# mcogoni/supersdr

Hardware: AMD Instinct MI355X
Metric: real-time IQ channels sustained (WF+demod) (higher is better)
Workload: dtype f32

## Files before the change

### supersdr_amd/csrc/ssdr_audio_dev.h

```cpp
#pragma once
#include "ssdr_math.h"
#include "ssdr_kernels.h"

constexpr int OCT = 10;
constexpr int NOCT = (SSDR_HIST + SSDR_FRAME) / 8;
constexpr int HOCT = SSDR_HIST / 8;
typedef uint32_t u32x4 __attribute__((ext_vector_type(4)));

SSDR_DEV void lds_sync()
{
    __builtin_amdgcn_fence(__ATOMIC_RELEASE, "wavefront");
    __builtin_amdgcn_wave_barrier();
    __builtin_amdgcn_fence(__ATOMIC_ACQUIRE, "wavefront");
}

template <int CTRL, int ROWMASK>
SSDR_DEV float dpp(float identity, float x)
{
    return __int_as_float(__builtin_amdgcn_update_dpp(__float_as_int(identity), __float_as_int(x), CTRL, ROWMASK, 0xF, false));
}
SSDR_DEV float vmax(float a, float b)
{
    float r;
    asm("v_max_f32 %0, %1, %2" : "=v"(r) : "v"(a), "v"(b));
    return r;
}
SSDR_DEV float vmax3(float a, float b, float c)
{
    float r;
    asm("v_max3_f32 %0, %1, %2, %3" : "=v"(r) : "v"(a), "v"(b), "v"(c));
    return r;
}
SSDR_DEV float vmax3_abs(float a, float b, float c)
{
    float r;
    asm("v_max3_f32 %0, %1, |%2|, |%3|" : "=v"(r) : "v"(a), "v"(b), "v"(c));
    return r;
}
SSDR_DEV uint32_t lane63_u(uint32_t x) { return (uint32_t)__builtin_amdgcn_readlane((int)x, 63); }
SSDR_DEV uint32_t from_prev_lane_u(uint32_t lane0_value, uint32_t x)
{
    return (uint32_t)__builtin_amdgcn_update_dpp((int)lane0_value, (int)x, 0x138, 0xF, 0xF, false);
}
typedef short s16x2 __attribute__((ext_vector_type(2)));
typedef unsigned short u16x2 __attribute__((ext_vector_type(2)));
SSDR_DEV uint32_t iq_power(uint32_t raw)
{
    uint32_t p;
    asm("v_dot2_i32_i16 %0, %1, %1, 0" : "=v"(p) : "v"(raw));
    return p;
}
SSDR_DEV float lane63(float x) { return __int_as_float(__builtin_amdgcn_readlane(__float_as_int(x), 63)); }
SSDR_DEV float from_prev_lane(float lane0_value, float x) { return dpp<0x138, 0xF>(lane0_value, x); }

#define SSDR_SCAN6(STEP) STEP("row_shr:1", "0xf") STEP("row_shr:2", "0xf") STEP("row_shr:4", "0xf") STEP("row_shr:8", "0xf") \
                         STEP("row_bcast:15", "0xa") STEP("row_bcast:31", "0xc")
#define SSDR_DPP(C, M) " " C " row_mask:" M " bank_mask:0xf"

SSDR_DEV float scan_max(float x)
{
#define STEP(C, M) asm("s_nop 1\n\tv_max_f32_dpp %0, %0, %0" SSDR_DPP(C, M) : "+v"(x));
    SSDR_SCAN6(STEP)
#undef STEP
    return x;
}
SSDR_DEV float scan_sum(float x)
{
#define STEP(C, M) asm("s_nop 1\n\tv_add_f32_dpp %0, %0, %0" SSDR_DPP(C, M) : "+v"(x));
    SSDR_SCAN6(STEP)
#undef STEP
    return x;
}
SSDR_DEV void scan_affine(float &A, float &B)
{
#define STEP(C, M) asm("s_nop 1\n\tv_fmac_f32_dpp %1, %1, %0" SSDR_DPP(C, M) "\n\tv_mul_f32_dpp %0, %0, %0" SSDR_DPP(C, M) : "+v"(A), "+v"(B));
    SSDR_SCAN6(STEP)
#undef STEP
}

struct Nco {
    uint32_t dphi;
    float cs, ss;
    float qc, qs;
    float tc, ts;
};
SSDR_DEV void nco_setup(Nco &n, uint32_t dphi, int l, int block = 8)
{
    n.dphi = dphi;
    ssdr_phasor32(dphi, n.cs, n.ss);
    ssdr_phasor32((uint32_t)(block * l) * dphi, n.qc, n.qs);
    n.tc = 1.0f; n.ts = 0.0f;
}
SSDR_DEV void nco_frame_table(Nco &n, uint32_t phase_of_frame, int l, int frame = SSDR_FRAME)
{
    ssdr_phasor32(phase_of_frame + (uint32_t)(frame * l) * n.dphi, n.tc, n.ts);
}
SSDR_DEV float lane_f(float x, uint32_t lane) { return __int_as_float(__builtin_amdgcn_readlane(__float_as_int(x), (int)lane)); }
SSDR_DEV void nco_block(const Nco &n, uint32_t f, float &c, float &s)
{
    const float fc = lane_f(n.tc, f & 63u), fs = lane_f(n.ts, f & 63u);
    c = fmaf(fc, n.qc, -(fs * n.qs));
    s = fmaf(fs, n.qc, fc * n.qs);
}
SSDR_DEV void phasor_mul(float ac, float as, float bc, float bs, float &c, float &s)
{
    c = fmaf(ac, bc, -(as * bs));
    s = fmaf(as, bc, ac * bs);
}

template <bool CLIP, int N = 8>
SSDR_DEV void mix8(const uint32_t (&rw)[N], float c, float s, float cs, float ss, float2 (&z)[N], float &amax)
{
#pragma unroll
    for (int j = 0; j < N; j++) {
        const float xr = (float)(int16_t)(rw[j] & 0xFFFFu);
        const float xi = (float)((int32_t)rw[j] >> 16);
        if (CLIP) amax = vmax3_abs(amax, xr, xi);
        z[j] = make_float2(fmaf(xr, c, xi * s), fmaf(xi, c, -(xr * s)));
        const float cn = fmaf(c, cs, -(s * ss)), sn = fmaf(s, cs, c * ss);
        c = cn; s = sn;
    }
}

template <bool CLIP>
SSDR_DEV void mix8_carry(const uint32_t *rw, float &c, float &s, float cs, float ss, float2 (&z)[8], float &amax)
{
#pragma unroll
    for (int j = 0; j < 8; j++) {
        const float xr = (float)(int16_t)(rw[j] & 0xFFFFu);
        const float xi = (float)((int32_t)rw[j] >> 16);
        if (CLIP) amax = vmax3_abs(amax, xr, xi);
        z[j] = make_float2(fmaf(xr, c, xi * s), fmaf(xi, c, -(xr * s)));
        const float cn = fmaf(c, cs, -(s * ss)), sn = fmaf(s, cs, c * ss);
        c = cn; s = sn;
    }
}

SSDR_DEV void load_oct(const float2 *z, int q, float2 (&v)[8])
{
    const float4 *p = reinterpret_cast<const float4 *>(z + q * OCT);
#pragma unroll
    for (int i = 0; i < 4; i++) {
        const float4 t = p[i];
        v[2 * i] = make_float2(t.x, t.y);
        v[2 * i + 1] = make_float2(t.z, t.w);
    }
}

SSDR_DEV void store_oct(float2 *z, int q, const float2 (&v)[8])
{
    float4 *p = reinterpret_cast<float4 *>(z + q * OCT);
#pragma unroll
    for (int i = 0; i < 4; i++) p[i] = make_float4(v[2 * i].x, v[2 * i].y, v[2 * i + 1].x, v[2 * i + 1].y);
}

template <int K0, int NK>
SSDR_DEV void fir_taps(const float *h, const float2 (&A)[8], const float2 (&B)[8], float (&yr)[8], float (&yi)[8])
{
#pragma unroll
    for (int kk = K0; kk < K0 + NK; kk++) {
#pragma unroll
        for (int j = 0; j < 8; j++) {
            const float2 v = (j - kk >= 0) ? A[(j - kk) & 7] : B[(8 + j - kk) & 7];
            yr[j] = fmaf(h[kk], v.x, yr[j]);
            yi[j] = fmaf(h[kk], v.y, yi[j]);
        }
    }
}


struct AgcK { float c0, c1, knee, d8; uint32_t K; };

template <bool INTEGER_POWER>
SSDR_DEV void demod_am(const float (&p)[8], float &dc, float (&aud)[8])
{
    constexpr float DC_APOW[8] = SSDR_DC_APOW_INIT;
    float env[8], loc[8];
    float s = 0.0f;
#pragma unroll
    for (int j = 0; j < 8; j++) {
        env[j] = INTEGER_POWER ? ssdr_sqrt_rn_int(p[j]) : ssdr_sqrt_rn(p[j]);
        s = fmaf(SSDR_DC_A, s, SSDR_DC_AL * env[j]);
        loc[j] = s;
    }
    float Asc = DC_APOW[7], Bsc = s;
    scan_affine(Asc, Bsc);
    const float Ae = from_prev_lane(1.0f, Asc), Be = from_prev_lane(0.0f, Bsc);
    const float carry = fmaf(Ae, dc, Be);
    float m = 0.0f;
#pragma unroll
    for (int j = 0; j < 8; j++) {
        m = fmaf(DC_APOW[j], carry, loc[j]);
        aud[j] = env[j] - m;
    }
    dc = lane63(m);
}

SSDR_DEV void demod_ssb(const float (&yr)[8], const float (&yi)[8], float c, float s, float cs2, float ss2, float (&aud)[8])
{
#pragma unroll
    for (int j = 0; j < 8; j++) {
        aud[j] = fmaf(yr[j], c, -(yi[j] * s));
        const float cn = fmaf(c, cs2, -(s * ss2)), sn = fmaf(s, cs2, c * ss2);
        c = cn; s = sn;
    }
}

SSDR_DEV void demod_fm(const float (&yr)[8], const float (&yi)[8], float prev_re, float prev_im, float kfm, float (&aud)[8])
{
    float pr = from_prev_lane(prev_re, yr[7]), pi = from_prev_lane(prev_im, yi[7]);
#pragma unroll
    for (int j = 0; j < 8; j++) {
        const float dr = fmaf(yr[j], pr, yi[j] * pi);
        const float di = fmaf(yi[j], pr, -(yr[j] * pi));
        aud[j] = ssdr_atan2p(di, dr) * kfm;
        pr = yr[j]; pi = yi[j];
    }
}

SSDR_DEV float block_peak(const float (&p)[8])
{
    return vmax3(vmax3(vmax3(p[0], p[1], p[2]), p[3], p[4]), vmax3(p[5], p[6], p[7]), SSDR_P_FLOOR);
}

SSDR_DEV float agc_pack_store(const float (&p)[8], const float (&aud)[8], int l, const AgcK &k, float &agc_d,
                              float (&agc_m)[8], int16_t *dst, float pm_known = -1.0f)
{
    const float pm = pm_known >= 0.0f ? pm_known : block_peak(p);
    const float al = ssdr_log2p(pm);
    const float fl = (float)l;
    const float d8 = k.d8;
    float e;
    if (k.K == 0) {
        const float P = scan_max(fmaf(fl, d8, al));
        e = vmax(fmaf(-fl, d8, P), fmaf(-(fl + 1.0f), d8, agc_d));
        agc_d = lane63(e);
    } else {
        const float P = scan_max(al);
        float maxM = agc_m[0], mK = agc_m[0];
#pragma unroll
        for (int i = 1; i < 8; i++)
            if ((uint32_t)i < k.K) { maxM = fmaxf(maxM, agc_m[i]); mK = agc_m[i]; }
        e = vmax(vmax(P, maxM), fmaf(-(fl + 1.0f), d8, agc_d));
        agc_d = fmaxf(fmaf(-64.0f, d8, agc_d), mK);
#pragma unroll
        for (int i = 7; i > 0; i--) agc_m[i] = agc_m[i - 1];
        agc_m[0] = lane63(P);
    }
    const float g = ssdr_exp2p(fmaf(k.c1, vmax(e, k.knee), k.c0));
    u32x4 w;
#pragma unroll
    for (int j = 0; j < 8; j += 2) {
        const int i0 = __float2int_rn(aud[j] * g), i1 = __float2int_rn(aud[j + 1] * g);
        w[j >> 1] = __builtin_bit_cast(uint32_t, __builtin_amdgcn_cvt_pk_i16(i0, i1));
    }
    SSDR_NT_STORE(w, reinterpret_cast<u32x4 *>(dst));
    return g;
}

SSDR_DEV void iq_pack_store(const float (&yr)[8], const float (&yi)[8], float g, uint32_t *dst)
{
    u32x4 w0, w1;
#pragma unroll
    for (int j = 0; j < 8; j++) {
        const uint32_t v = __builtin_bit_cast(uint32_t, __builtin_amdgcn_cvt_pk_i16(__float2int_rn(yr[j] * g), __float2int_rn(yi[j] * g)));
        if (j < 4) w0[j] = v; else w1[j - 4] = v;
    }
    SSDR_NT_STORE(w0, reinterpret_cast<u32x4 *>(dst));
    SSDR_NT_STORE(w1, reinterpret_cast<u32x4 *>(dst) + 1);
}

SSDR_DEV void rssi_flag_step(const float (&p)[8], bool clip, uint32_t f, uint32_t n_frames, int l, float cal,
                             float &rssi_sum, uint32_t &flag_keep, float *rssi_row, uint8_t *flag_row)
{
    float ps = p[0];
#pragma unroll
    for (int j = 1; j < 8; j++) ps = ps + p[j];
    const float tot = lane63(scan_sum(ps));
    if ((f & 63u) == (uint32_t)l) { rssi_sum = tot; flag_keep = clip ? 1u : 0u; }
    if ((f & 63u) == 63u || f + 1 == n_frames) {
        if ((uint32_t)l <= (f & 63u)) {
            rssi_row[(f & ~63u) + l] = fmaf(ssdr_log2p(fmaxf(rssi_sum, 1e-20f)) - 39.0f, SSDR_DB_PER_LOG2, cal);
            flag_row[(f & ~63u) + l] = (uint8_t)flag_keep;
        }
    }
}

SSDR_DEV bool wave_any(bool x) { return __builtin_amdgcn_ballot_w64(x) != 0ull; }

SSDR_DEV bool raw_clipped(const uint32_t (&rw)[8])
{
    bool c = false;
#pragma unroll
    for (int j = 0; j < 8; j++) {
        const int lo = (int16_t)(rw[j] & 0xFFFFu), hi = (int32_t)rw[j] >> 16;
        c = c || lo >= 32767 || lo <= -32767 || hi >= 32767 || hi <= -32767;
    }
    return c;
}

SSDR_DEV uint32_t scan_add_u(uint32_t x)
{
#define STEP(C, M) asm("s_nop 1\n\tv_add_u32_dpp %0, %0, %0" SSDR_DPP(C, M) : "+v"(x));
    SSDR_SCAN6(STEP)
#undef STEP
    return x;
}
SSDR_DEV uint32_t scan_max_u(uint32_t x)
{
#define STEP(C, M) asm("s_nop 1\n\tv_max_u32_dpp %0, %0, %0" SSDR_DPP(C, M) : "+v"(x));
    SSDR_SCAN6(STEP)
#undef STEP
    return x;
}

struct NbRun { uint32_t gate, thresh, s1, s2, left; };

template <int N>
SSDR_DEV uint32_t nb_frame(uint32_t (&rw)[N], int l, NbRun &s, bool &clip)
{
    constexpr uint32_t M = 64u * N;
    constexpr int SHIFT = __builtin_ctz(M);
    const uint32_t lmin = s.s1 < s.s2 ? s.s1 : s.s2;
    const uint64_t t64 = (uint64_t)s.thresh * lmin;
    const uint32_t tc = (t64 == 0 || t64 >= 0xFFFFFFFFull) ? 0xFFFFFFFFu : (uint32_t)t64;
    uint32_t part = 0, trig = 0;
    u16x2 rails = {0xFFFFu, 0xFFFFu};
#pragma unroll
    for (int j = 0; j < N; j++) {
        const uint32_t p = iq_power(rw[j]);
        part += p >> SHIFT;
        trig |= (uint32_t)(p > tc) << j;
        rails = __builtin_elementwise_min(rails, __builtin_bit_cast(u16x2, rw[j]) + (u16x2){32769u, 32769u});
    }
    clip = wave_any(rails.x < 3u || rails.y < 3u);
    const uint32_t n0 = (uint32_t)(N * l);
    const uint32_t le = trig ? n0 + (31u - (uint32_t)__builtin_clz(trig)) + s.gate : 0u;
    const uint32_t sc = scan_max_u(le);
    const uint32_t from_left = from_prev_lane_u(0u, sc);
    const uint32_t e = s.left > from_left ? s.left : from_left;
    int d = (int)e - (int)n0;
    uint32_t mask = 0;
#pragma unroll
    for (int j = 0; j < N; j++) {
        d = (trig >> j) & 1u ? j + (int)s.gate : d;
        const bool b = j < d;
        mask |= (uint32_t)b << j;
        rw[j] = b ? 0u : rw[j];
    }
    const uint32_t sum = lane63_u(scan_add_u(part));
    const uint32_t last = lane63_u(sc);
    const uint32_t ef = s.left > last ? s.left : last;
    s.left = ef > M ? ef - M : 0u;
    s.s2 = s.s1;
    s.s1 = sum;
    return mask;
}
```

### supersdr_amd/csrc/ssdr_wf.hip

```cpp
#include "ssdr_math.h"
#include "ssdr_kernels.h"
#include "ssdr_audio_dev.h"
#include "ssdr_wf_dev.h"

namespace {

constexpr int WAVES = SSDR_WF_BLOCK / 64;
constexpr int LDS_TOTAL = LDS_XCH + WAVES * 2 * XCH_FLOATS * 4;
static_assert(LDS_TOTAL <= 163840, "LDS budget");

template <bool AVG, bool HOP>
__global__ __launch_bounds__(SSDR_WF_BLOCK, SSDR_WF_WAVES_PER_EU) void ssdr_wf_kernel(SsdrWfArgs a)
{
    __shared__ __attribute__((aligned(16))) unsigned char smem[LDS_TOTAL];
    load_tables(smem, a.win, a.tw_stage, a.lut);

    const int lane = threadIdx.x & 63, wave = __builtin_amdgcn_readfirstlane(threadIdx.x >> 6);
    const int h = lane >> 5, l = lane & 31;
    float *xch_wave = reinterpret_cast<float *>(smem + LDS_XCH) + wave * 2 * XCH_FLOATS;
    const unsigned char *lut = smem + LDS_LUT0;
    const uint32_t n_pairs = (a.n_ch + 1) >> 1;
    const uint32_t run = HOP ? a.grp_run : 1u;
    const uint32_t n_runs = (a.n_groups + run - 1) / run;
    const uint32_t n_items = n_pairs * n_runs;
    const uint32_t wave_stride = gridDim.x * WAVES;

    for (uint32_t item = blockIdx.x * WAVES + wave; item < n_items; item += wave_stride) {
      uint32_t pair, g_begin, g_end;
      if (HOP) {
          pair = item / n_runs;
          g_begin = (item - pair * n_runs) * run;
          g_end = min(g_begin + run, a.n_groups);
      } else {
          g_begin = item / n_pairs;
          pair = item - g_begin * n_pairs;
          g_end = g_begin + 1;
      }
      const uint32_t n_trips = HOP ? g_end - g_begin : 1u;
      for (uint32_t trip = 0; trip < n_trips; trip++) {
        const uint32_t grp = g_begin + trip;
        uint32_t pair_now = __builtin_amdgcn_readfirstlane(pair);
        asm volatile("" : "+s"(pair_now));
        const WfItem it = wf_item(a, pair_now, grp, h);
        const float calq = a.consts[it.ch].wf_cal_lin * SSDR_LUT_SCALE;
        uint32_t acc[AVG ? 16 : 1];
#pragma unroll
        for (int j = 0; j < (AVG ? 16 : 1); j++) acc[j] = 0;
        constexpr uint32_t LINE_STEP = HOP ? SSDR_NFFT / 2 : SSDR_NFFT;
        const uint32_t *src = a.iq + (uint64_t)it.ch * a.ch_stride + (uint64_t)it.l0 * LINE_STEP + l;

        for (uint32_t line = it.l0; line < it.l1; line++, src += LINE_STEP) {
            f32x2 z[32];
            uint32_t raw[32];
            if (HOP) load_line_halves(line ? src - SSDR_NFFT / 2 : a.tail + (uint64_t)it.ch * (SSDR_NFFT / 2) + l, src, raw);
            else load_line(src, raw);
            if (SSDR_PRIO_WF) prio_compute_phase();
            window_line(raw, smem, l, z);
            SCHED_FENCE();
            fft_line<AVG>(z, smem, xch_wave, h, l);
            if (SSDR_PRIO_WF) prio_latency_phase();

            if (AVG) {
                quantise32(z, calq, lut, [&](int j, uint32_t q01) { acc[j] += q01; });
            } else {
                uint32_t q[16];
                quantise32(z, calq, lut, [&](int j, uint32_t q01) { q[j] = q01; });
                int16_t *x16 = reinterpret_cast<int16_t *>(xch_wave + opaque(h) * XCH_FLOATS) + opaque(l);
#pragma unroll
                for (int j = 0; j < 16; j++) {
                    x16[32 * (j + 16)] = (int16_t)(q[j] & 0xFFFFu);
                    x16[32 * j] = (int16_t)(q[j] >> 16);
                }
            }
        }

        float *xch = xch_wave + opaque(h) * XCH_FLOATS;
        if (AVG) {
            int16_t *x16 = reinterpret_cast<int16_t *>(xch) + opaque(l);
#pragma unroll
            for (int j = 0; j < 16; j++) {
                x16[32 * (j + 16)] = (int16_t)(acc[j] & 0xFFFFu);
                x16[32 * j] = (int16_t)(acc[j] >> 16);
            }
        }
        wave_lds_sync();
        const u32x4 *x128 = reinterpret_cast<const u32x4 *>(xch);
        int16_t *dst = it.complete ? a.out + ((uint64_t)it.grp * a.n_ch + it.ch) * SSDR_NFFT
                                   : a.acc_out + (uint64_t)it.ch * SSDR_NFFT;
        const int16_t *cin = a.acc_in + (uint64_t)it.ch * SSDR_NFFT;
#pragma unroll
        for (int q = 0; q < 4; q++) {
            u32x4 v = x128[q * 32 + l];
            if (AVG && it.carry_in)
                v += reinterpret_cast<const u32x4 *>(cin)[q * 32 + l];
            if (it.ch_ok) SSDR_NT_STORE(v, reinterpret_cast<u32x4 *>(dst) + q * 32 + l);
        }
        wave_lds_sync();
      }
    }
}

template <bool HOP, bool AVG = false>
__global__ __launch_bounds__(SSDR_WF_BLOCK, SSDR_WF_WAVES_PER_EU) void ssdr_fused_am_kernel(SsdrFusedArgs fa)
{
    __shared__ __attribute__((aligned(16))) unsigned char smem[LDS_TOTAL];
    const SsdrWfArgs &a = fa.wf;
    const SsdrAudioArgs &u = fa.au;
    load_tables(smem, a.win, a.tw_stage, a.lut);

    const int lane = threadIdx.x & 63, wave = __builtin_amdgcn_readfirstlane(threadIdx.x >> 6);
    const int h = lane >> 5, l = lane & 31;
    float *xch_wave = reinterpret_cast<float *>(smem + LDS_XCH) + wave * 2 * XCH_FLOATS;
    uint32_t *qbuf = reinterpret_cast<uint32_t *>(xch_wave);
    const unsigned char *lut = smem + LDS_LUT0;
    const uint32_t n_pairs = (a.n_ch + 1) >> 1;
    const uint32_t wave_stride = gridDim.x * WAVES;
    const uint32_t n_frames = u.n_frames;

    for (uint32_t pair = blockIdx.x * WAVES + wave; pair < n_pairs; pair += wave_stride) {
        const uint32_t ch_raw = 2 * pair + h;
        const bool ch_ok = ch_raw < a.n_ch;
        const uint32_t ch = ch_ok ? ch_raw : a.n_ch - 1;
        const float cal_wf = a.consts[ch].wf_cal_lin * SSDR_LUT_SCALE;
        const uint32_t n_sub = (2 * pair + 1 < a.n_ch) ? 2u : 1u;

        float rssi_sum[2] = {0.0f, 0.0f};
        uint32_t flag_keep[2] = {0u, 0u};
        auto pad = [&](int c, int i) -> float & { return xch_wave[c * XCH_FLOATS + 33 * (i + 16) + 32]; };
        if (lane < 2) {
            const uint32_t cc = min(2 * pair + (uint32_t)lane, a.n_ch - 1);
            const ssdr_chan_state st = u.state[cc];
            pad(lane, 0) = st.dc;
            pad(lane, 1) = st.agc_d;
#pragma unroll
            for (int i = 0; i < 8; i++) pad(lane, 2 + i) = st.agc_m[i];
            const uint4 t = *reinterpret_cast<const uint4 *>(u.hist + (size_t)cc * SSDR_HIST + SSDR_HIST - 4);
            pad(lane, 10) = __uint_as_float(iq_power(t.x)); pad(lane, 11) = __uint_as_float(iq_power(t.y));
            pad(lane, 12) = __uint_as_float(iq_power(t.z)); pad(lane, 13) = __uint_as_float(iq_power(t.w));
        }
        wave_lds_sync();

        const uint32_t *src = a.iq + (uint64_t)ch * a.ch_stride + l;
        uint32_t last_raw31 = 0;
        uint32_t acc[AVG ? 16 : 1];
#pragma unroll
        for (int j = 0; j < (AVG ? 16 : 1); j++) acc[j] = 0;
        constexpr uint32_t LINE_STEP = HOP ? SSDR_NFFT / 2 : SSDR_NFFT;
        constexpr int FRAMES_PER_LINE = HOP ? 1 : 2;
        for (uint32_t line = 0; line < a.n_lines; line++, src += LINE_STEP) {
            float dc[2], agc_d[2], agc_m[2][8];
            uint32_t tail_q[2][4];
#pragma unroll
            for (int c = 0; c < 2; c++) {
                dc[c] = pad(c, 0); agc_d[c] = pad(c, 1);
#pragma unroll
                for (int i = 0; i < 8; i++) agc_m[c][i] = pad(c, 2 + i);
#pragma unroll
                for (int i = 0; i < 4; i++) tail_q[c][i] = __float_as_uint(pad(c, 10 + i));
            }
            wave_lds_sync();
            {
                const uint32_t lw = opaque(lane);
                u32x4 t[2][4];
#pragma unroll
                for (int c = 0; c < 2; c++) {
                    uint32_t pair_now = __builtin_amdgcn_readfirstlane(pair);
                    asm volatile("" : "+s"(pair_now));
                    const uint32_t cc = min(2 * pair_now + (uint32_t)c, a.n_ch - 1);
                    const uint32_t *row = a.iq + (uint64_t)cc * a.ch_stride + (uint64_t)line * LINE_STEP;
                    if (HOP) {
                        const uint32_t *older = line ? row - SSDR_NFFT / 2 : a.tail + (uint64_t)cc * (SSDR_NFFT / 2);
#pragma unroll
                        for (int i = 0; i < 2; i++) t[c][i] = SSDR_NT_LOAD(reinterpret_cast<const u32x4 *>(older) + 64 * i + lw);
#pragma unroll
                        for (int i = 0; i < 2; i++) t[c][2 + i] = reinterpret_cast<const u32x4 *>(row)[64 * i + lw];
                    } else {
#pragma unroll
                        for (int i = 0; i < 4; i++) t[c][i] = SSDR_NT_LOAD(reinterpret_cast<const u32x4 *>(row) + 64 * i + lw);
                    }
                }
                SCHED_FENCE();
#pragma unroll
                for (int c = 0; c < 2; c++)
#pragma unroll
                    for (int i = 0; i < 4; i++) reinterpret_cast<u32x4 *>(qbuf + c * XCH_FLOATS)[64 * i + lw] = t[c][i];
                SCHED_FENCE();
            }
            wave_lds_sync();
            prio_latency_phase();
#pragma unroll
            for (int c = 0; c < 2; c++) {
                if ((uint32_t)c >= n_sub) continue;
                uint32_t pair_now = __builtin_amdgcn_readfirstlane(pair);
                asm volatile("" : "+s"(pair_now));
                const uint32_t cc = 2 * pair_now + c;
                const ssdr_chan_consts &kc = u.consts[cc];
                const AgcK agc_c = {kc.agc_c0, kc.agc_c1, kc.agc_knee, kc.agc_delta8, kc.hang_frames};
                const float cal_c = kc.smeter_cal_db;
#pragma unroll
                for (int f = 0; f < FRAMES_PER_LINE; f++) {
                    const uint32_t frame = HOP ? line : 2 * line + f;
                    const u32x4 *qp = reinterpret_cast<const u32x4 *>(qbuf + c * XCH_FLOATS + SSDR_FRAME * (HOP ? 1 : f)) + 2 * opaque(lane);
                    const u32x4 q0 = qp[0], q1 = qp[1];
                    const uint32_t rw[8] = {q0.x, q0.y, q0.z, q0.w, q1.x, q1.y, q1.z, q1.w};
                    uint32_t qv[8], d[8];
#pragma unroll
                    for (int j = 0; j < 8; j++) qv[j] = iq_power(rw[j]);
                    float p[8], aud[8];
#pragma unroll
                    for (int j = 0; j < 4; j++) { d[j] = from_prev_lane_u(tail_q[c][j], qv[4 + j]); d[4 + j] = qv[j]; }
#pragma unroll
                    for (int j = 0; j < 4; j++) tail_q[c][j] = lane63_u(qv[4 + j]);
#pragma unroll
                    for (int j = 0; j < 8; j++) p[j] = (float)d[j];
                    const float pmx = block_peak(p);
                    const bool trig = wave_any(pmx >= 1073676160.0f) || tail_q[c][0] >= 0x3FFF0001u || tail_q[c][1] >= 0x3FFF0001u ||
                                      tail_q[c][2] >= 0x3FFF0001u || tail_q[c][3] >= 0x3FFF0001u;
                    const bool clip = trig ? wave_any(raw_clipped(rw)) : false;
                    demod_am<true>(p, dc[c], aud);
                    agc_pack_store(p, aud, lane, agc_c, agc_d[c], agc_m[c], u.pcm + ((uint64_t)cc * n_frames + frame) * SSDR_FRAME + 8 * lane, pmx);
                    rssi_flag_step(p, clip, frame, n_frames, lane, cal_c, rssi_sum[c], flag_keep[c],
                                   u.rssi + (uint64_t)cc * n_frames, u.flags + (uint64_t)cc * n_frames);
                }
            }
            wave_lds_sync();
            prio_compute_phase();
            uint32_t raw[32];
            {
                const uint32_t *q = qbuf + opaque(h) * XCH_FLOATS + opaque(l);
#pragma unroll
                for (int r = 0; r < 32; r++) raw[r] = q[32 * r];
            }
            wave_lds_sync();
            if (lane < 2) {
#pragma unroll
                for (int c = 0; c < 2; c++) {
                    if (lane != c) continue;
                    pad(c, 0) = dc[c]; pad(c, 1) = agc_d[c];
#pragma unroll
                    for (int i = 0; i < 8; i++) pad(c, 2 + i) = agc_m[c][i];
#pragma unroll
                    for (int i = 0; i < 4; i++) pad(c, 10 + i) = __uint_as_float(tail_q[c][i]);
                }
            }
            wave_lds_sync();
            SCHED_FENCE();
            if (line + 1 == a.n_lines && ch_ok) {
#pragma unroll
                for (int r = 28; r < 32; r++) u.hist[(size_t)ch * SSDR_HIST + 32 * (r - 28) + l] = raw[r];
            }
            last_raw31 = raw[31];
            uint32_t qn[16];
            f32x2 z[32];
            window_line(raw, smem, l, z);
            SCHED_FENCE();
            fft_line<true>(z, smem, xch_wave, h, l);
            prio_latency_phase();
            if (AVG) quantise32(z, cal_wf, lut, [&](int j, uint32_t q01) { acc[j] += q01; });
            else quantise32(z, cal_wf, lut, [&](int j, uint32_t q01) { qn[j] = q01; });
            const uint32_t pos = a.phase + line;
            const bool group_done = !AVG || (pos + 1) % a.n_avg == 0;
            const bool last_line = line + 1 == a.n_lines;
            if (group_done || last_line) {
                float *xch = xch_wave + opaque(h) * XCH_FLOATS;
                int16_t *x16 = reinterpret_cast<int16_t *>(xch) + opaque(l);
#pragma unroll
                for (int j = 0; j < 16; j++) {
                    const uint32_t v = AVG ? acc[j] : qn[j];
                    x16[32 * (j + 16)] = (int16_t)(v & 0xFFFFu);
                    x16[32 * j] = (int16_t)(v >> 16);
                }
                wave_lds_sync();
                const u32x4 *x128 = reinterpret_cast<const u32x4 *>(xch);
                const uint32_t grp = AVG ? pos / a.n_avg : line;
                int16_t *dst = group_done ? a.out + ((uint64_t)grp * a.n_ch + ch) * SSDR_NFFT : a.acc_out + (uint64_t)ch * SSDR_NFFT;
                const bool carry_in = AVG && grp == 0 && a.phase != 0;
                const int16_t *cin = a.acc_in + (uint64_t)ch * SSDR_NFFT;
#pragma unroll
                for (int q = 0; q < 4; q++) {
                    u32x4 v = x128[q * 32 + l];
                    if (carry_in) v += reinterpret_cast<const u32x4 *>(cin)[q * 32 + l];
                    if (ch_ok) SSDR_NT_STORE(v, reinterpret_cast<u32x4 *>(dst) + q * 32 + l);
                }
                wave_lds_sync();
                if (AVG) {
#pragma unroll
                    for (int j = 0; j < 16; j++) acc[j] = 0;
                }
            }
        }

        if (a.n_lines) {
#pragma unroll
            for (int c = 0; c < 2; c++) {
                if ((uint32_t)c >= n_sub) continue;
                const uint32_t cc = 2 * pair + c;
                const ssdr_chan_consts &kc = u.consts[cc];
                ssdr_chan_state st = u.state[cc];
                const uint32_t phi_last = st.phi1 + (uint32_t)(SSDR_FRAME * (n_frames - 1)) * kc.dphi1;
                float fc, fs, qc, qs, bc, bs, cs, ss;
                ssdr_phasor32(phi_last, fc, fs);
                ssdr_phasor32((uint32_t)(8 * 63) * kc.dphi1, qc, qs);
                ssdr_phasor32(kc.dphi1, cs, ss);
                phasor_mul(fc, fs, qc, qs, bc, bs);
#pragma unroll
                for (int j = 0; j < 3; j++) { const float cn = fmaf(bc, cs, -(bs * ss)), sn = fmaf(bs, cs, bc * ss); bc = cn; bs = sn; }
                const float xr = (float)(int16_t)(last_raw31 & 0xFFFFu), xi = (float)((int32_t)last_raw31 >> 16);
                const float zr = fmaf(xr, bc, xi * bs) + 0.0f, zi = fmaf(xi, bc, -(xr * bs)) + 0.0f;
                st.prev_re = lane_f(zr, 32 * c + 27);
                st.prev_im = lane_f(zi, 32 * c + 27);
                st.phi1 += (uint32_t)(SSDR_FRAME * n_frames) * kc.dphi1;
                st.phi2 += (uint32_t)(SSDR_FRAME * n_frames) * kc.dphi2;
                st.dc = pad(c, 0); st.agc_d = pad(c, 1);
#pragma unroll
                for (int i = 0; i < 8; i++) st.agc_m[i] = pad(c, 2 + i);
                if (lane == 0) u.state[cc] = st;
            }
        }
    }
}

__global__ __launch_bounds__(256) void ssdr_quant_selftest_kernel(const float *thr_g, const uint32_t *lut_g,
                                                                    unsigned long long *mismatch)
{
    __shared__ __attribute__((aligned(16))) unsigned char smem[LDS_LUT_END + 16 + 1024];
    float *s_thr = reinterpret_cast<float *>(smem + ((LDS_LUT_END + 15) & ~15));
    uint32_t *s_lut = reinterpret_cast<uint32_t *>(smem + LDS_LUT0);
    for (int i = threadIdx.x; i < 256; i += blockDim.x) s_thr[i] = thr_g[i];
    for (int i = threadIdx.x; i < SSDR_LUT_N; i += blockDim.x) s_lut[i] = lut_g[i];
    __syncthreads();
    unsigned long long bad = 0;
    const unsigned char *lut = smem + LDS_LUT0;
    const uint64_t stride = (uint64_t)gridDim.x * blockDim.x;
    for (uint64_t u = (uint64_t)blockIdx.x * blockDim.x + threadIdx.x; u < 0x7F800000ull; u += stride) {
        const float p = __uint_as_float((uint32_t)u);
        int lo = 0, hi = 255;
        while (lo < hi) {
            const int mid = (lo + hi + 1) >> 1;
            if (s_thr[mid] <= p) lo = mid; else hi = mid - 1;
        }
        float pc;
        asm("v_mul_f32_e64 %0, %1, %2 clamp" : "=v"(pc) : "v"(p), "v"(SSDR_LUT_SCALE));
        bad += (quantise(pc, lut) != (uint32_t)lo);
    }
    if (bad) atomicAdd(mismatch, bad);
}

}

hipError_t ssdr_launch_wf(const SsdrWfArgs &a, uint32_t grid, hipStream_t stream)
{
    const dim3 g(grid), b(SSDR_WF_BLOCK);
    if (a.tail) {
        if (a.n_avg > 1) hipLaunchKernelGGL((ssdr_wf_kernel<true, true>), g, b, 0, stream, a);
        else hipLaunchKernelGGL((ssdr_wf_kernel<false, true>), g, b, 0, stream, a);
    } else {
        if (a.n_avg > 1) hipLaunchKernelGGL((ssdr_wf_kernel<true, false>), g, b, 0, stream, a);
        else hipLaunchKernelGGL((ssdr_wf_kernel<false, false>), g, b, 0, stream, a);
    }
    return hipGetLastError();
}

hipError_t ssdr_launch_fused_am(const SsdrFusedArgs &a, uint32_t grid, hipStream_t stream)
{
    if (a.wf.n_avg > 1) {
        if (a.wf.tail) hipLaunchKernelGGL((ssdr_fused_am_kernel<true, true>), dim3(grid), dim3(SSDR_WF_BLOCK), 0, stream, a);
        else hipLaunchKernelGGL((ssdr_fused_am_kernel<false, true>), dim3(grid), dim3(SSDR_WF_BLOCK), 0, stream, a);
    } else {
        if (a.wf.tail) hipLaunchKernelGGL((ssdr_fused_am_kernel<true, false>), dim3(grid), dim3(SSDR_WF_BLOCK), 0, stream, a);
        else hipLaunchKernelGGL((ssdr_fused_am_kernel<false, false>), dim3(grid), dim3(SSDR_WF_BLOCK), 0, stream, a);
    }
    return hipGetLastError();
}

hipError_t ssdr_fused_blocks_per_cu(int *blocks)
{
    int b[4] = {0, 0, 0, 0};
    hipError_t e = hipOccupancyMaxActiveBlocksPerMultiprocessor(&b[0], ssdr_fused_am_kernel<false, false>, SSDR_WF_BLOCK, 0);
    if (e == hipSuccess) e = hipOccupancyMaxActiveBlocksPerMultiprocessor(&b[1], ssdr_fused_am_kernel<true, false>, SSDR_WF_BLOCK, 0);
    if (e == hipSuccess) e = hipOccupancyMaxActiveBlocksPerMultiprocessor(&b[2], ssdr_fused_am_kernel<false, true>, SSDR_WF_BLOCK, 0);
    if (e == hipSuccess) e = hipOccupancyMaxActiveBlocksPerMultiprocessor(&b[3], ssdr_fused_am_kernel<true, true>, SSDR_WF_BLOCK, 0);
    *blocks = b[0];
    for (int i = 1; i < 4; i++) *blocks = b[i] < *blocks ? b[i] : *blocks;
    return e;
}

hipError_t ssdr_wf_blocks_per_cu(int *blocks)
{
    int b[4] = {0, 0, 0, 0};
    hipError_t e = hipOccupancyMaxActiveBlocksPerMultiprocessor(&b[0], ssdr_wf_kernel<false, false>, SSDR_WF_BLOCK, 0);
    if (e == hipSuccess) e = hipOccupancyMaxActiveBlocksPerMultiprocessor(&b[1], ssdr_wf_kernel<true, false>, SSDR_WF_BLOCK, 0);
    if (e == hipSuccess) e = hipOccupancyMaxActiveBlocksPerMultiprocessor(&b[2], ssdr_wf_kernel<false, true>, SSDR_WF_BLOCK, 0);
    if (e == hipSuccess) e = hipOccupancyMaxActiveBlocksPerMultiprocessor(&b[3], ssdr_wf_kernel<true, true>, SSDR_WF_BLOCK, 0);
    if (e != hipSuccess) return e;
    *blocks = b[0];
    for (int i = 1; i < 4; i++) *blocks = b[i] < *blocks ? b[i] : *blocks;
    return hipSuccess;
}

hipError_t ssdr_launch_quant_selftest(const float *thr, const uint32_t *lut, unsigned long long *mismatch, hipStream_t stream)
{
    hipLaunchKernelGGL(ssdr_quant_selftest_kernel, dim3(2048), dim3(256), 0, stream, thr, lut, mismatch);
    return hipGetLastError();
}
```

Before: 43.88 million.

## Keep AM demod AGC/DC carry state in scalar registers and a dedicated LDS slot

The per-channel DC, AGC decay and tail-power carries used to be saved to and reloaded from the LDS exchange pad on every line, which cost extra wave barriers. They are now held in wave-uniform scalar registers (readfirstlane plus asm pinning), and the 8-entry AGC hang history moves to its own small LDS region read as float4. This removes a load/sync and a store/sync per line and replaces the runtime-indexed hang loop with a switch over fixed window sizes. The cost is more LDS per workgroup, still checked against a two-workgroup-per-CU budget, and more SGPR pressure.

```diff
diff --git a/supersdr_amd/csrc/ssdr_audio_dev.h b/supersdr_amd/csrc/ssdr_audio_dev.h
--- a/supersdr_amd/csrc/ssdr_audio_dev.h
+++ b/supersdr_amd/csrc/ssdr_audio_dev.h
@@ -258,6 +258,63 @@
     return g;
 }
 
+SSDR_DEV uint32_t uni_u(uint32_t x) { return (uint32_t)__builtin_amdgcn_readfirstlane((int)x); }
+SSDR_DEV float uni(float x) { return __uint_as_float(uni_u(__float_as_uint(x))); }
+
+struct AgcCarryU { float d; float *m; };
+
+template <int KK>
+SSDR_DEV void hang_window(const float (&m)[8], float &maxM, float &mK)
+{
+    maxM = m[0];
+#pragma unroll
+    for (int i = 1; i < KK; i++) maxM = fmaxf(maxM, m[i]);
+    mK = m[KK - 1];
+}
+
+SSDR_DEV float agc_pack_store(const float (&p)[8], const float (&aud)[8], int l, const AgcK &k, AgcCarryU &s, int16_t *dst, float pm)
+{
+    const uint32_t K = uni_u(k.K);
+    const float al = ssdr_log2p(pm);
+    const float fl = (float)l;
+    const float d8 = k.d8;
+    float e;
+    if (K == 0) {
+        const float P = scan_max(fmaf(fl, d8, al));
+        e = vmax(fmaf(-fl, d8, P), fmaf(-(fl + 1.0f), d8, s.d));
+        s.d = lane63(e);
+    } else {
+        const float P = scan_max(al);
+        float4 *m4 = reinterpret_cast<float4 *>(s.m);
+        const float4 a = m4[0], b = m4[1];
+        const float m[8] = {a.x, a.y, a.z, a.w, b.x, b.y, b.z, b.w};
+        float maxM, mK;
+        switch (K) {
+        case 1: hang_window<1>(m, maxM, mK); break;
+        case 2: hang_window<2>(m, maxM, mK); break;
+        case 3: hang_window<3>(m, maxM, mK); break;
+        case 4: hang_window<4>(m, maxM, mK); break;
+        case 5: hang_window<5>(m, maxM, mK); break;
+        case 6: hang_window<6>(m, maxM, mK); break;
+        case 7: hang_window<7>(m, maxM, mK); break;
+        default: hang_window<8>(m, maxM, mK); break;
+        }
+        e = vmax(vmax(P, maxM), fmaf(-(fl + 1.0f), d8, s.d));
+        s.d = uni(fmaxf(fmaf(-64.0f, d8, s.d), mK));
+        m4[0] = make_float4(lane63(P), a.x, a.y, a.z);
+        m4[1] = make_float4(a.w, b.x, b.y, b.z);
+    }
+    const float g = ssdr_exp2p(fmaf(k.c1, vmax(e, k.knee), k.c0));
+    u32x4 w;
+#pragma unroll
+    for (int j = 0; j < 8; j += 2) {
+        const int i0 = __float2int_rn(aud[j] * g), i1 = __float2int_rn(aud[j + 1] * g);
+        w[j >> 1] = __builtin_bit_cast(uint32_t, __builtin_amdgcn_cvt_pk_i16(i0, i1));
+    }
+    SSDR_NT_STORE(w, reinterpret_cast<u32x4 *>(dst));
+    return g;
+}
+
 SSDR_DEV void iq_pack_store(const float (&yr)[8], const float (&yi)[8], float g, uint32_t *dst)
 {
     u32x4 w0, w1;
diff --git a/supersdr_amd/csrc/ssdr_wf.hip b/supersdr_amd/csrc/ssdr_wf.hip
--- a/supersdr_amd/csrc/ssdr_wf.hip
+++ b/supersdr_amd/csrc/ssdr_wf.hip
@@ -8,6 +8,22 @@
 constexpr int WAVES = SSDR_WF_BLOCK / 64;
 constexpr int LDS_TOTAL = LDS_XCH + WAVES * 2 * XCH_FLOATS * 4;
 static_assert(LDS_TOTAL <= 163840, "LDS budget");
+constexpr int LDS_AGCM = LDS_TOTAL;
+constexpr int LDS_TOTAL_FUSED = LDS_AGCM + WAVES * 2 * 8 * 4;
+static_assert(LDS_AGCM % 16 == 0 && 2 * LDS_TOTAL_FUSED <= 163840, "LDS budget: two workgroups per CU");
+
+SSDR_DEV void keep_scalar(uint32_t &x)
+{
+    uint32_t s = uni_u(x);
+    asm volatile("" : "+s"(s));
+    x = s;
+}
+SSDR_DEV void keep_scalar(float &x)
+{
+    uint32_t s = __float_as_uint(x);
+    keep_scalar(s);
+    x = __uint_as_float(s);
+}
 
 template <bool AVG, bool HOP>
 __global__ __launch_bounds__(SSDR_WF_BLOCK, SSDR_WF_WAVES_PER_EU) void ssdr_wf_kernel(SsdrWfArgs a)
@@ -103,7 +119,7 @@
 template <bool HOP, bool AVG = false>
 __global__ __launch_bounds__(SSDR_WF_BLOCK, SSDR_WF_WAVES_PER_EU) void ssdr_fused_am_kernel(SsdrFusedArgs fa)
 {
-    __shared__ __attribute__((aligned(16))) unsigned char smem[LDS_TOTAL];
+    __shared__ __attribute__((aligned(16))) unsigned char smem[LDS_TOTAL_FUSED];
     const SsdrWfArgs &a = fa.wf;
     const SsdrAudioArgs &u = fa.au;
     load_tables(smem, a.win, a.tw_stage, a.lut);
@@ -126,17 +142,22 @@
 
         float rssi_sum[2] = {0.0f, 0.0f};
         uint32_t flag_keep[2] = {0u, 0u};
-        auto pad = [&](int c, int i) -> float & { return xch_wave[c * XCH_FLOATS + 33 * (i + 16) + 32]; };
-        if (lane < 2) {
-            const uint32_t cc = min(2 * pair + (uint32_t)lane, a.n_ch - 1);
+        float dc[2], agc_d[2];
+        uint32_t tail_q[2][4];
+        float *agc_m = reinterpret_cast<float *>(smem + LDS_AGCM) + wave * 16;
+#pragma unroll
+        for (int c = 0; c < 2; c++) {
+            const uint32_t cc = min(2 * pair + (uint32_t)c, a.n_ch - 1);
             const ssdr_chan_state st = u.state[cc];
-            pad(lane, 0) = st.dc;
-            pad(lane, 1) = st.agc_d;
-#pragma unroll
-            for (int i = 0; i < 8; i++) pad(lane, 2 + i) = st.agc_m[i];
+            dc[c] = uni(st.dc);
+            agc_d[c] = uni(st.agc_d);
+            if (lane == 0) {
+#pragma unroll
+                for (int i = 0; i < 8; i++) agc_m[8 * c + i] = st.agc_m[i];
+            }
             const uint4 t = *reinterpret_cast<const uint4 *>(u.hist + (size_t)cc * SSDR_HIST + SSDR_HIST - 4);
-            pad(lane, 10) = __uint_as_float(iq_power(t.x)); pad(lane, 11) = __uint_as_float(iq_power(t.y));
-            pad(lane, 12) = __uint_as_float(iq_power(t.z)); pad(lane, 13) = __uint_as_float(iq_power(t.w));
+            tail_q[c][0] = uni_u(iq_power(t.x)); tail_q[c][1] = uni_u(iq_power(t.y));
+            tail_q[c][2] = uni_u(iq_power(t.z)); tail_q[c][3] = uni_u(iq_power(t.w));
         }
         wave_lds_sync();
 
@@ -148,17 +169,6 @@
         constexpr uint32_t LINE_STEP = HOP ? SSDR_NFFT / 2 : SSDR_NFFT;
         constexpr int FRAMES_PER_LINE = HOP ? 1 : 2;
         for (uint32_t line = 0; line < a.n_lines; line++, src += LINE_STEP) {
-            float dc[2], agc_d[2], agc_m[2][8];
-            uint32_t tail_q[2][4];
-#pragma unroll
-            for (int c = 0; c < 2; c++) {
-                dc[c] = pad(c, 0); agc_d[c] = pad(c, 1);
-#pragma unroll
-                for (int i = 0; i < 8; i++) agc_m[c][i] = pad(c, 2 + i);
-#pragma unroll
-                for (int i = 0; i < 4; i++) tail_q[c][i] = __float_as_uint(pad(c, 10 + i));
-            }
-            wave_lds_sync();
             {
                 const uint32_t lw = opaque(lane);
                 u32x4 t[2][4];
@@ -218,10 +228,18 @@
                                       tail_q[c][2] >= 0x3FFF0001u || tail_q[c][3] >= 0x3FFF0001u;
                     const bool clip = trig ? wave_any(raw_clipped(rw)) : false;
                     demod_am<true>(p, dc[c], aud);
-                    agc_pack_store(p, aud, lane, agc_c, agc_d[c], agc_m[c], u.pcm + ((uint64_t)cc * n_frames + frame) * SSDR_FRAME + 8 * lane, pmx);
+                    AgcCarryU carry = {agc_d[c], agc_m + 8 * c};
+                    agc_pack_store(p, aud, lane, agc_c, carry, u.pcm + ((uint64_t)cc * n_frames + frame) * SSDR_FRAME + 8 * lane, pmx);
+                    agc_d[c] = carry.d;
                     rssi_flag_step(p, clip, frame, n_frames, lane, cal_c, rssi_sum[c], flag_keep[c],
                                    u.rssi + (uint64_t)cc * n_frames, u.flags + (uint64_t)cc * n_frames);
                 }
+            }
+#pragma unroll
+            for (int c = 0; c < 2; c++) {
+                keep_scalar(dc[c]); keep_scalar(agc_d[c]);
+#pragma unroll
+                for (int j = 0; j < 4; j++) keep_scalar(tail_q[c][j]);
             }
             wave_lds_sync();
             prio_compute_phase();
@@ -230,18 +248,6 @@
                 const uint32_t *q = qbuf + opaque(h) * XCH_FLOATS + opaque(l);
 #pragma unroll
                 for (int r = 0; r < 32; r++) raw[r] = q[32 * r];
-            }
-            wave_lds_sync();
-            if (lane < 2) {
-#pragma unroll
-                for (int c = 0; c < 2; c++) {
-                    if (lane != c) continue;
-                    pad(c, 0) = dc[c]; pad(c, 1) = agc_d[c];
-#pragma unroll
-                    for (int i = 0; i < 8; i++) pad(c, 2 + i) = agc_m[c][i];
-#pragma unroll
-                    for (int i = 0; i < 4; i++) pad(c, 10 + i) = __uint_as_float(tail_q[c][i]);
-                }
             }
             wave_lds_sync();
             SCHED_FENCE();
@@ -311,9 +317,9 @@
                 st.prev_im = lane_f(zi, 32 * c + 27);
                 st.phi1 += (uint32_t)(SSDR_FRAME * n_frames) * kc.dphi1;
                 st.phi2 += (uint32_t)(SSDR_FRAME * n_frames) * kc.dphi2;
-                st.dc = pad(c, 0); st.agc_d = pad(c, 1);
-#pragma unroll
-                for (int i = 0; i < 8; i++) st.agc_m[i] = pad(c, 2 + i);
+                st.dc = dc[c]; st.agc_d = agc_d[c];
+#pragma unroll
+                for (int i = 0; i < 8; i++) st.agc_m[i] = agc_m[8 * c + i];
                 if (lane == 0) u.state[cc] = st;
             }
         }
```

New measurement: 44.13 million (median of 6 runs). No clear change (+0.6%).
